# ilpoviertola/V-AURA

Measured on AMD Instinct MI355X. Metric: audio codec tokens/sec (whole node), 2.56 s clips, higher is better.
Workload: dtype f16x2-split(22b)/f32-acc

## Files before the change

### vaura_amd/csrc/dac.hip

```cpp
#include "common.h"
#include <algorithm>
#include <vector>

#define BM 128
#define BN 96
#define BK 32

struct ConvArgs {
  const float* in;
  const float* w;
  const float* bias;
  const float* res;
  const float* alpha;
  float* out_raw;
  float* out_act;
  int Lin, Lout, Cin, Cout, NT;
  int off_base, off_step;
  int ostride, oshift0;
  int jcount;
};

__host__ __device__ __forceinline__ size_t mx8_scale_offset(size_t elems) { return (elems + 15) & ~(size_t)15; }

#ifndef VA_CONV_ABL
// ... 128 lines not shown
  int off_base, off_step, ostride, oshift0, jcount;
  int act;
  int act_fmt;
  uint8_t* out_scale;
  const uint32_t* in_scale;
  const float* wscale;
  const uint16_t* w2;
  const float* bias2;
  const float* alpha_mid;
};

__device__ __forceinline__ float gelu_erf_f(float x) {
  if constexpr ((VA_CONV_ABL & 128) != 0) return 0.5f * x * (1.0f + x * 0.70710678118654752440f);
  if constexpr ((VA_CONV_ABL & 256) != 0) return 0.5f * x * (1.0f + erff(x * 0.70710678118654752440f));
  const float t = fabsf(x) * 0.70710678118654752440f;
  const float k = __builtin_amdgcn_rcpf(fmaf(t, 0.35f, 1.0f));
  float p = 0.06797561794519424f;
  p = fmaf(p, k, -0.4044332206249237f);
  p = fmaf(p, k, 0.8392713069915771f);
  p = fmaf(p, k, -0.7225478887557983f);
  p = fmaf(p, k, 0.6403822898864746f);
  p = fmaf(p, k, -0.046077974140644073f);
  p = fmaf(p, k, 0.23748238384723663f);
  p = fmaf(p, k, 0.1900186985731125f);
  p = fmaf(p, k, 0.1979287713766098f);
  const float e = (k * p) * __builtin_amdgcn_exp2f(-(t * t) * 1.4426950408889634f);
  return (0.5f * x) * (x < 0.f ? e : 2.0f - e);
}

__device__ __forceinline__ void store_pair4(uint16_t* base, size_t row, int c0, int C, const f32x4 v) {
  _Float16 h[4], l[4];
#pragma unroll
  for (int i = 0; i < 4; ++i) {
    const float x = v[i];
    h[i] = (_Float16)x;
    l[i] = (_Float16)(x - (float)h[i]);
  }
  typedef _Float16 f16x4 __attribute__((ext_vector_type(4)));
  f16x4* p = reinterpret_cast<f16x4*>(base + ((row * (size_t)(C >> 3) + (size_t)(c0 >> 3)) * 2) * 8 + (c0 & 7));
  p[0] = f16x4{h[0], h[1], h[2], h[3]};
  p[2] = f16x4{l[0], l[1], l[2], l[3]};
}

__device__ __forceinline__ int mx8_scale_byte(float amax) {
  const uint32_t bits = __builtin_bit_cast(uint32_t, amax);
  const int ea = (int)((bits >> 23) & 0xffu);
  const int e8 = ea - ((bits & 0x7fffffu) <= 0x600000u ? 8 : 7);
  return e8 < 1 ? 1 : (e8 > 253 ? 253 : e8);
}

__device__ __forceinline__ void store_act_octet(void* out_act, uint8_t* out_scale, int fmt, size_t grow, int co, int C,
                                                const float (&sv)[8]) {
  if (fmt == 0) {
    f16x8 hi, lo;
#pragma unroll
    for (int r = 0; r < 8; ++r) { hi[r] = (_Float16)sv[r]; lo[r] = (_Float16)(sv[r] - (float)hi[r]); }
    f16x8* dst = reinterpret_cast<f16x8*>(reinterpret_cast<uint16_t*>(out_act) + ((grow * (size_t)(C >> 3) + (size_t)(co >> 3)) * 2) * 8);
    dst[0] = hi;
    dst[1] = lo;
  } else {
    float amax = 0.f;
#pragma unroll
    for (int r = 0; r < 8; ++r) amax = fmaxf(amax, fabsf(sv[r]));
    amax = fmaxf(amax, __shfl_xor(amax, 1, 64));
    amax = fmaxf(amax, __shfl_xor(amax, 2, 64));
    const int e8 = mx8_scale_byte(amax);
    const float inv = __builtin_bit_cast(float, (uint32_t)(254 - e8) << 23);
    int q0 = 0, q1 = 0;
    q0 = __builtin_amdgcn_cvt_pk_fp8_f32(sv[0] * inv, sv[1] * inv, q0, false);
    q0 = __builtin_amdgcn_cvt_pk_fp8_f32(sv[2] * inv, sv[3] * inv, q0, true);
    q1 = __builtin_amdgcn_cvt_pk_fp8_f32(sv[4] * inv, sv[5] * inv, q1, false);
    q1 = __builtin_amdgcn_cvt_pk_fp8_f32(sv[6] * inv, sv[7] * inv, q1, true);
    typedef int i32x2 __attribute__((ext_vector_type(2)));
    *reinterpret_cast<i32x2*>(reinterpret_cast<uint8_t*>(out_act) + grow * (size_t)C + co) = i32x2{q0, q1};
    if (((co >> 3) & 3) == 0) out_scale[(grow * (size_t)((C + 127) >> 7) + (co >> 7)) * 4 + ((co >> 5) & 3)] = (uint8_t)e8;
  }
}

__device__ __forceinline__ float snake_fast(float v, float al) {
  const float sn = __builtin_amdgcn_sinf(__builtin_amdgcn_fractf(al * v * 0.15915494309189535f));
  return v + __builtin_amdgcn_rcpf(al + 1e-9f) * (sn * sn);
}

template <int BN_, int SP, bool FAST = false, int ROWS = BM>
__device__ __forceinline__ void conv_tile_store(const ConvPArgs& a, const float* stage, int b, int ph, int j0, int n0, int tid) {
  constexpr int OCT = BN_ / 8;
  static_assert(OCT % 4 == 0, "a 32-channel scale block = 4 consecutive threads of one row");
  constexpr int RSTEP = 256 / OCT;
  if (tid >= RSTEP * OCT) return;
  const int oc = tid % OCT, row0 = tid / OCT;
  const int co = n0 + oc * 8;
  const size_t obase = (size_t)b * a.Lout;
  f32x4 al0 = f32x4{0.f, 0.f, 0.f, 0.f}, al1 = al0, iv0 = al0, iv1 = al0;
  if (a.out_act && a.act == 0) {
    al0 = *reinterpret_cast<const f32x4*>(a.alpha + co);
    al1 = *reinterpret_cast<const f32x4*>(a.alpha + co + 4);
#pragma unroll
    for (int r = 0; r < 4; ++r) { iv0[r] = 1.0f / (al0[r] + 1e-9f); iv1[r] = 1.0f / (al1[r] + 1e-9f); }
  }
  for (int row = row0; row < ROWS; row += RSTEP) {
    const int jr = j0 + row;
    if (jr >= a.jcount) continue;
    const int orow = jr * a.ostride + a.oshift0 + ph;
    if (orow < 0 || orow >= a.Lout) continue;
    const size_t o = (obase + (size_t)orow) * a.Cout + co;
    f32x4 v0 = *reinterpret_cast<const f32x4*>(stage + row * SP + oc * 8);
    f32x4 v1 = *reinterpret_cast<const f32x4*>(stage + row * SP + oc * 8 + 4);
    if (a.res) {
      v0 = *reinterpret_cast<const f32x4*>(a.res + o) + v0;
      v1 = *reinterpret_cast<const f32x4*>(a.res + o + 4) + v1;
    }
    if (a.out_raw) {
      *reinterpret_cast<f32x4*>(a.out_raw + o) = v0;
      *reinterpret_cast<f32x4*>(a.out_raw + o + 4) = v1;
    }
    if (a.out_act) {
      float sv[8];
#pragma unroll
      for (int r = 0; r < 4; ++r) {
        if (FAST && a.act == 0) {
          sv[r] = snake_fast(v0[r], al0[r]);
          sv[r + 4] = snake_fast(v1[r], al1[r]);
        } else {
          sv[r] = a.act == 0 ? snake_fi(v0[r], al0[r], iv0[r]) : (a.act == 1 ? gelu_erf_f(v0[r]) : v0[r]);
          sv[r + 4] = a.act == 0 ? snake_fi(v1[r], al1[r], iv1[r]) : (a.act == 1 ? gelu_erf_f(v1[r]) : v1[r]);
        }
      }
      store_act_octet(a.out_act, a.out_scale, a.act_fmt, obase + (size_t)orow, co, a.Cout, sv);
    }
  }
}

#define XHALO 56
#define XROWS (BM + XHALO)
#ifndef VA_CONV_ABL
#define VA_CONV_ABL 0
#endif
template <int NI, bool WS, bool XS = false, int MJ = 4, bool FUSE = false>
__global__ __launch_bounds__(256, 2) void conv_pair_kernel(ConvPArgs a) {
  constexpr int BN_ = 32 * NI;
  constexpr int BMT = 32 * MJ;
  constexpr int XROWS_T = BMT + XHALO;
  constexpr int NXB = MJ == 4 ? 2 : 1;
  static_assert(MJ == 4 || MJ == 8, "128 or 256 rows");
  constexpr int WSTR = (BN_ + 3 + 15) / 16 * 16, XSTR = (XROWS_T + 3 + 15) / 16 * 16;
  constexpr int WS_ELEMS = 2 * (BK / 4) * WSTR, XS_ELEMS = NXB * (BK / 4) * XSTR;
  constexpr int SP = BN_ + 4;
  static_assert((WS_ELEMS + XS_ELEMS) * 16 >= BM * SP * 4, "the output tile must fit in the main loop's LDS");
  static_assert(!FUSE || (NI == 3 && MJ == 8), "the fused residual unit: all 96 channels in one 256-row workgroup");
  constexpr int W1STR = 112, YSTR = 80;
  constexpr int W1_ELEMS = FUSE ? 3 * (BK / 4) * W1STR : 0, Y_ELEMS = FUSE ? 3 * (BK / 4) * YSTR : 0;
  static_assert(!FUSE || Y_ELEMS * 16 >= 64 * SP * 4, "the 64-row output tile is staged over the activated tile");
  constexpr int SMEM_ELEMS = (WS_ELEMS + XS_ELEMS) > (W1_ELEMS + Y_ELEMS) ? (WS_ELEMS + XS_ELEMS) : (W1_ELEMS + Y_ELEMS);
  constexpr int TAB_ELEMS = FUSE ? 2 * BN_ / 4 : 0;
  __shared__ u32x4 smem[SMEM_ELEMS + TAB_ELEMS];
  auto coff = [](int kq) { return (kq & 1) + ((kq >> 2) << 1); };
  auto Ws = [&](int buf, int kq, int row) -> u32x4& { return smem[(buf * (BK / 4) + kq) * WSTR + row + coff(kq)]; };
  auto Xs = [&](int buf, int kq, int row) -> u32x4& { return smem[WS_ELEMS + (buf * (BK / 4) + kq) * XSTR + row + coff(kq)]; };
  const int tid = threadIdx.x, lane = tid & 63, wv = tid >> 6;
  const int wn = wv & 1, wm = wv >> 1;
  const int j0 = blockIdx.x * BMT;
  const int n0 = blockIdx.y * BN_;
  const int phases = a.ostride;
  const int b = blockIdx.z / phases, ph = blockIdx.z % phases;
  const int cq = a.Cin / 4;
  const u32x4* in = reinterpret_cast<const u32x4*>(a.in) + (size_t)b * a.Lin * cq;
  const u32x4* wbase = reinterpret_cast<const u32x4*>(a.w) + (size_t)ph * a.NT * a.Cout * cq;
  const int kc = a.Cin / BK;
  const int NT = a.NT;
  const int nk = NT * kc;
  const int span = (NT - 1) * (a.off_step < 0 ? -a.off_step : a.off_step);
  const int lo_off = a.off_base + (a.off_step < 0 ? (NT - 1) * a.off_step : 0);
  const int xrows = BMT + span;
  constexpr int XL = (XROWS_T * (BK / 4) + 255) / 256;

  u32x4 wreg[NI], xreg[XL];
  auto load_w = [&](int kt) {
    const int c = kt / NT, t = kt - c * NT;
    const u32x4* wt = wbase + (size_t)t * a.Cout * cq;
    const int q0 = c * (BK / 4);
#pragma unroll
    for (int i = 0; i < NI; ++i) {
      const int qd = tid + 256 * i, row = qd >> 3, kq = qd & 7;
      wreg[i] = wt[(size_t)(n0 + row) * cq + q0 + kq];
    }
  };
  auto store_w = [&](int buf) {
#pragma unroll
    for (int i = 0; i < NI; ++i) { const int qd = tid + 256 * i; Ws(buf, qd & 7, qd >> 3) = wreg[i]; }
  };
  auto load_x = [&](int c) {
    const int q0 = c * (BK / 4);
#pragma unroll
    for (int i = 0; i < XL; ++i) {
      const int qd = tid + 256 * i, row = qd >> 3, kq = qd & 7;
      const int jr = j0 + lo_off + row;
      xreg[i] = (row < xrows && jr >= 0 && jr < a.Lin) ? in[(size_t)jr * cq + q0 + kq] : u32x4{0u, 0u, 0u, 0u};
    }
  };
  auto store_x = [&](int buf) {
#pragma unroll
    for (int i = 0; i < XL; ++i) {
      const int qd = tid + 256 * i;
      if ((qd >> 3) < XROWS_T) Xs(buf, qd & 7, qd >> 3) = xreg[i];
    }
  };

  f32x4 acc[NI][MJ];
#pragma unroll
  for (int i = 0; i < NI; ++i)
#pragma unroll
    for (int j = 0; j < MJ; ++j) acc[i][j] = f32x4{0.f, 0.f, 0.f, 0.f};

  VA_STAMP_DECL(stamps);
  VA_STAMP(stamps, 0);
  load_w(0);
  load_x(0);
  store_w(0);
  store_x(0);
  if constexpr (FUSE) {
    if (tid < BN_) {
      float* tab = reinterpret_cast<float*>(smem + SMEM_ELEMS);
      const float al = a.alpha_mid[tid];
      tab[tid] = al;
      tab[BN_ + tid] = 1.0f / (al + 1e-9f);
    }
  }
  __syncthreads();
  VA_STAMP(stamps, 1);
  const int g = lane >> 4, r16 = lane & 15;
  int kt = 0;
  for (int c = 0; c < kc; ++c) {
    const int xb = NXB == 2 ? (c & 1) : 0;
    for (int t = 0; t < NT; ++t, ++kt) {
      const int buf = kt & 1;
      if (kt + 1 < nk && !(VA_CONV_ABL & 1)) load_w(kt + 1);
      if (t == (NXB == 2 ? 0 : NT - 1) && c + 1 < kc) load_x(c + 1);
      const int shift = (VA_CONV_ABL & 8) ? 0 : a.off_base + t * a.off_step - lo_off;
      f16x8 wh[NI], wl[NI];
#pragma unroll
      for (int i = 0; i < NI; ++i) {
        wh[i] = __builtin_bit_cast(f16x8, Ws(buf, 2 * g, wn * (NI * 16) + i * 16 + r16));
        if constexpr (!WS && !XS) wl[i] = __builtin_bit_cast(f16x8, Ws(buf, 2 * g + 1, wn * (NI * 16) + i * 16 + r16));
      }
      constexpr int JG = MJ == 4 ? 4 : 2;
#pragma unroll
      for (int jh = 0; jh < MJ; jh += JG) {
        f16x8 xh[JG], xl[JG];
#pragma unroll
        for (int j = 0; j < JG; ++j) {
          xh[j] = __builtin_bit_cast(f16x8, Xs(xb, 2 * g, shift + wm * (16 * MJ) + (jh + j) * 16 + r16));
          if constexpr (!XS) xl[j] = __builtin_bit_cast(f16x8, Xs(xb, 2 * g + 1, shift + wm * (16 * MJ) + (jh + j) * 16 + r16));
        }
#pragma unroll
        for (int i = 0; i < NI; ++i)
#pragma unroll
          for (int j = 0; j < JG; ++j) {
            if constexpr (VA_CONV_ABL & 2) {
              acc[i][jh + j][0] += (float)wh[i][0] * (float)xh[j][0];
              if constexpr (!XS) acc[i][jh + j][1] += (float)xl[j][0];
              if constexpr (!WS && !XS) acc[i][jh + j][2] += (float)wl[i][0];
              continue;
            }
            if constexpr (!WS && !XS) acc[i][jh + j] = __builtin_amdgcn_mfma_f32_16x16x32_f16(wl[i], xh[j], acc[i][jh + j], 0, 0, 0);
            if constexpr (!XS) acc[i][jh + j] = __builtin_amdgcn_mfma_f32_16x16x32_f16(wh[i], xl[j], acc[i][jh + j], 0, 0, 0);
            acc[i][jh + j] = __builtin_amdgcn_mfma_f32_16x16x32_f16(wh[i], xh[j], acc[i][jh + j], 0, 0, 0);
          }
      }
      if (kt + 1 < nk && !(VA_CONV_ABL & 1)) store_w(buf ^ 1);
      if (t == NT - 1 && c + 1 < kc) {
        if constexpr (NXB == 1) __syncthreads();
        store_x(NXB == 2 ? (xb ^ 1) : 0);
      }
      if constexpr (!(VA_CONV_ABL & 4)) __syncthreads();
    }
  }

  VA_STAMP(stamps, 2);
  if constexpr (FUSE) {
    u32x4* W1 = smem;
    u32x4* Yi = smem + W1_ELEMS;
    auto W1s = [&](int c2, int kq, int row) -> u32x4& { return W1[(c2 * (BK / 4) + kq) * W1STR + row + coff(kq)]; };
    auto Ys = [&](int c2, int kq, int row) -> u32x4& { return Yi[(c2 * (BK / 4) + kq) * YSTR + row + coff(kq)]; };
    u32x4 w1reg[9];
#pragma unroll
    for (int i = 0; i < 9; ++i) w1reg[i] = reinterpret_cast<const u32x4*>(a.w2)[tid + 256 * i];
    float* stage = reinterpret_cast<float*>(Yi);
    const float* tab = reinterpret_cast<const float*>(smem + SMEM_ELEMS);
    typedef _Float16 f16x4 __attribute__((ext_vector_type(4)));
    auto pass = [&](auto pc) {
      constexpr int p = decltype(pc)::value;
      if (p > 0) __syncthreads();
      if (wm == (p >> 1)) {
#pragma unroll
        for (int jj = 0; jj < 4; ++jj)
#pragma unroll
          for (int i = 0; i < NI; ++i) {
            const int col = wn * (NI * 16) + i * 16 + 4 * g;
            const f32x4 v = acc[i][4 * (p & 1) + jj] + *reinterpret_cast<const f32x4*>(a.bias + col);
            const f32x4 al = *reinterpret_cast<const f32x4*>(tab + col), iv = *reinterpret_cast<const f32x4*>(tab + BN_ + col);
            f16x4 h4, l4;
#pragma unroll
            for (int e = 0; e < 4; ++e) {
              const float sv = snake_fi(v[e], al[e], iv[e]);
              h4[e] = (_Float16)sv;
              l4[e] = (_Float16)(sv - (float)h4[e]);
            }
            const int c2 = col >> 5, o = (col & 31) >> 3, half = (col & 7) >> 2, row = jj * 16 + r16;
            reinterpret_cast<f16x4*>(&Ys(c2, 2 * o, row))[half] = h4;
            reinterpret_cast<f16x4*>(&Ys(c2, 2 * o + 1, row))[half] = l4;
          }
      }
      if (p == 0) {
#pragma unroll
        for (int i = 0; i < 9; ++i) {
          const int qd = tid + 256 * i, n = qd / 24, q = qd - n * 24;
          W1s(q >> 3, q & 7, n) = w1reg[i];
        }
      }
      __syncthreads();
      if (p == 0) VA_STAMP(stamps, 3);
      f32x4 acc2[NI][2];
#pragma unroll
      for (int i = 0; i < NI; ++i)
#pragma unroll
        for (int j = 0; j < 2; ++j) acc2[i][j] = f32x4{0.f, 0.f, 0.f, 0.f};
#pragma unroll
      for (int c2 = 0; c2 < 3; ++c2) {
        f16x8 wh[NI], wl[NI], xh[2], xl[2];
#pragma unroll
        for (int i = 0; i < NI; ++i) {
          wh[i] = __builtin_bit_cast(f16x8, W1s(c2, 2 * g, wn * (NI * 16) + i * 16 + r16));
          if constexpr (!WS && !XS) wl[i] = __builtin_bit_cast(f16x8, W1s(c2, 2 * g + 1, wn * (NI * 16) + i * 16 + r16));
        }
#pragma unroll
        for (int j = 0; j < 2; ++j) {
          xh[j] = __builtin_bit_cast(f16x8, Ys(c2, 2 * g, (wm * 2 + j) * 16 + r16));
          if constexpr (!XS) xl[j] = __builtin_bit_cast(f16x8, Ys(c2, 2 * g + 1, (wm * 2 + j) * 16 + r16));
        }
#pragma unroll
        for (int i = 0; i < NI; ++i)
#pragma unroll
          for (int j = 0; j < 2; ++j) {
            if constexpr (!WS && !XS) acc2[i][j] = __builtin_amdgcn_mfma_f32_16x16x32_f16(wl[i], xh[j], acc2[i][j], 0, 0, 0);
            if constexpr (!XS) acc2[i][j] = __builtin_amdgcn_mfma_f32_16x16x32_f16(wh[i], xl[j], acc2[i][j], 0, 0, 0);
            acc2[i][j] = __builtin_amdgcn_mfma_f32_16x16x32_f16(wh[i], xh[j], acc2[i][j], 0, 0, 0);
          }
      }
      __syncthreads();
      if (p == 0) VA_STAMP(stamps, 4);
#pragma unroll
      for (int i = 0; i < NI; ++i)
#pragma unroll
        for (int j = 0; j < 2; ++j) {
          const int row = (wm * 2 + j) * 16 + r16, col = wn * (NI * 16) + i * 16 + 4 * g;
          *reinterpret_cast<f32x4*>(stage + row * SP + col) = acc2[i][j] + *reinterpret_cast<const f32x4*>(a.bias2 + col);
        }
      __syncthreads();
      conv_tile_store<BN_, SP, false, 64>(a, stage, b, ph, j0 + p * 64, n0, tid);
      if (p == 0) VA_STAMP(stamps, 5);
    };
    pass(std::integral_constant<int, 0>{});
    pass(std::integral_constant<int, 1>{});
    pass(std::integral_constant<int, 2>{});
    pass(std::integral_constant<int, 3>{});
    VA_STAMP(stamps, 6);
    VA_STAMP_FLUSH(stamps, 21);
    return;
  }
  float* stage = reinterpret_cast<float*>(smem);
#pragma unroll
  for (int h = 0; h < MJ / 4; ++h) {
    if (h > 0) __syncthreads();
#pragma unroll
    for (int j = 0; j < MJ; ++j) {
      const int rbk = wm * MJ + j;
      if (rbk / 8 != h) continue;
#pragma unroll
      for (int i = 0; i < NI; ++i) {
        const int row = (rbk % 8) * 16 + r16, col = wn * (NI * 16) + i * 16 + 4 * g;
        *reinterpret_cast<f32x4*>(stage + row * SP + col) = acc[i][j] + *reinterpret_cast<const f32x4*>(a.bias + n0 + col);
      }
    }
    __syncthreads();
    if (h == 0) VA_STAMP(stamps, 4);
    conv_tile_store<BN_, SP>(a, stage, b, ph, j0 + h * BM, n0, tid);
    if (h == 0) VA_STAMP(stamps, 5);
  }
  VA_STAMP(stamps, 6);
  VA_STAMP_FLUSH(stamps, 20);
}

template <int N, typename F>
__device__ __forceinline__ void va_static_for(F&& f) {
  if constexpr (N > 0) {
    va_static_for<N - 1>(f);
    f(std::integral_constant<int, N - 1>{});
  }
}

template <int NCT, int RB, bool WS, bool XS>
__global__ __launch_bounds__(256, 2) void conv_unit_kernel(ConvPArgs a) {
  constexpr int C_ = 16 * NCT;
  constexpr int BMT = 64 * RB;
  constexpr int KC = C_ / BK;
  constexpr int XROWS_T = BMT + XHALO;
  constexpr int WSTR = (C_ + 3 + 15) / 16 * 16, XSTR = (XROWS_T + 3 + 15) / 16 * 16, W2STR = (BN + 3 + 15) / 16 * 16;
  constexpr int WS_ELEMS = 2 * (BK / 4) * WSTR, XS_ELEMS = (BK / 4) * XSTR;
  constexpr int SP = BN + 4;
  constexpr int W2_ELEMS = 2 * (BK / 4) * W2STR, ST_ELEMS = 64 * SP / 4;
  constexpr int MAIN_ELEMS = WS_ELEMS + XS_ELEMS > W2_ELEMS + ST_ELEMS ? WS_ELEMS + XS_ELEMS : W2_ELEMS + ST_ELEMS;
  constexpr int TAB_ELEMS = 2 * C_ / 4;
  static_assert(NCT % 6 == 0 && (RB == 2 || RB == 4) && NCT * RB == 24, "96 channels x 256 rows or 192 x 128: 96 accumulator registers");
  __shared__ u32x4 smem[MAIN_ELEMS + TAB_ELEMS];
  auto coff = [](int kq) { return (kq & 1) + ((kq >> 2) << 1); };
  auto Ws = [&](int buf, int kq, int row) -> u32x4& { return smem[(buf * (BK / 4) + kq) * WSTR + row + coff(kq)]; };
  auto Xs = [&](int kq, int row) -> u32x4& { return smem[WS_ELEMS + kq * XSTR + row + coff(kq)]; };
  auto W2s = [&](int buf, int kq, int row) -> u32x4& { return smem[(buf * (BK / 4) + kq) * W2STR + row + coff(kq)]; };
  float* tab = reinterpret_cast<float*>(smem + MAIN_ELEMS);
  const int tid = threadIdx.x, lane = tid & 63;
  const int wv = __builtin_amdgcn_readfirstlane(tid >> 6);
  const int g = lane >> 4, r16 = lane & 15;
  const int j0 = blockIdx.x * BMT, b = blockIdx.z;
  constexpr int cq = C_ / 4;
  const u32x4* in = reinterpret_cast<const u32x4*>(a.in) + (size_t)b * a.Lin * cq;
  const u32x4* wbase = reinterpret_cast<const u32x4*>(a.w);
  const int NT = a.NT, nk = NT * KC;
  const int span = (NT - 1) * (a.off_step < 0 ? -a.off_step : a.off_step);
  const int lo_off = a.off_base + (a.off_step < 0 ? (NT - 1) * a.off_step : 0);
  const int xrows = BMT + span;
  constexpr int WL = C_ * (BK / 4) / 256;
  constexpr int XL = (XROWS_T * (BK / 4) + 255) / 256;

  u32x4 wreg[WL], xreg[XL];
  auto load_w = [&](int kt) {
    const int c = kt / NT, t = kt - c * NT;
    const u32x4* wt = wbase + (size_t)t * C_ * cq + c * (BK / 4);
#pragma unroll
    for (int i = 0; i < WL; ++i) { const int qd = tid + 256 * i; wreg[i] = wt[(size_t)(qd >> 3) * cq + (qd & 7)]; }
  };
  auto store_w = [&](int buf) {
#pragma unroll
    for (int i = 0; i < WL; ++i) {
      const int qd = tid + 256 * i, ch = qd >> 3, w5 = ch & 31;
      Ws(buf, qd & 7, (ch & ~31) + (((w5 >> 2) & 1) << 4) + ((w5 >> 3) << 2) + (w5 & 3)) = wreg[i];
    }
  };
  auto load_x = [&](int c) {
#pragma unroll
    for (int i = 0; i < XL; ++i) {
      const int qd = tid + 256 * i, row = qd >> 3, kq = qd & 7;
      const int jr = j0 + lo_off + row;
      xreg[i] = (row < xrows && jr >= 0 && jr < a.Lin) ? in[(size_t)jr * cq + c * (BK / 4) + kq] : u32x4{0u, 0u, 0u, 0u};
    }
  };
  auto store_x = [&]() {
#pragma unroll
    for (int i = 0; i < XL; ++i) { const int qd = tid + 256 * i; if ((qd >> 3) < XROWS_T) Xs(qd & 7, qd >> 3) = xreg[i]; }
  };

  f32x4 acc[NCT][RB];
#pragma unroll
  for (int i = 0; i < NCT; ++i)
#pragma unroll
    for (int j = 0; j < RB; ++j) acc[i][j] = f32x4{0.f, 0.f, 0.f, 0.f};

  VA_STAMP_DECL(stamps);
  VA_STAMP(stamps, 0);
  load_w(0);
  load_x(0);
  store_w(0);
  store_x();
  for (int ch = tid; ch < C_; ch += 256) {
// ... 403 lines not shown
      const f16x8* pp = reinterpret_cast<const f16x8*>(reinterpret_cast<const _Float16*>(act) + (((size_t)b * L + r) * oct + oc) * 16);
      const f16x8 h = pp[0], lo = pp[1];
#pragma unroll
      for (int e = 0; e < 8; ++e) x[e] = (float)h[e] + (float)lo[e];
    } else {
      const f32x4* pp = reinterpret_cast<const f32x4*>(act + ((size_t)b * L + r) * C + 8 * oc);
      const f32x4 a0 = pp[0], a1 = pp[1];
      x[0] = a0[0]; x[1] = a0[1]; x[2] = a0[2]; x[3] = a0[3]; x[4] = a1[0]; x[5] = a1[1]; x[6] = a1[2]; x[7] = a1[3];
    }
    *reinterpret_cast<f32x4*>(rows + rr * SR + 8 * oc) = f32x4{x[0], x[1], x[2], x[3]};
    *reinterpret_cast<f32x4*>(rows + rr * SR + 8 * oc + 4) = f32x4{x[4], x[5], x[6], x[7]};
  }
  __syncthreads();
  const int half = __builtin_amdgcn_readfirstlane(tid >> 7), lo_ = tid & 127;
  const int c0 = half * (C >> 1), c1 = c0 + (C >> 1);
  f32x4 d4 = f32x4{0.f, 0.f, 0.f, 0.f};
#pragma unroll
  for (int t = 0; t < 7; ++t) {
    const f32x4* xr = reinterpret_cast<const f32x4*>(rows + (lo_ + t) * SR + c0);
    const f32x4* wr = reinterpret_cast<const f32x4*>(w + (size_t)t * C + c0);
#pragma unroll 4
    for (int c = 0; c < (c1 - c0) / 4; ++c) {
      const f32x4 x = xr[c], ww = wr[c];
      d4[0] = fmaf(x[0], ww[0], d4[0]); d4[1] = fmaf(x[1], ww[1], d4[1]); d4[2] = fmaf(x[2], ww[2], d4[2]); d4[3] = fmaf(x[3], ww[3], d4[3]);
    }
  }
  const float d = (d4[0] + d4[1]) + (d4[2] + d4[3]);
  float* part = rows + (CO_TL + 6) * SR;
  if (half) part[lo_] = d;
  __syncthreads();
  if (!half && l0 + lo_ < L) wav[(size_t)b * L + l0 + lo_] = tanhf((d + part[lo_]) + bias[0]);
}

__global__ __launch_bounds__(256) void act_convert_kernel(const float* __restrict__ in, void* out, uint8_t* out_scale, size_t rows,
                                                          int C, int fmt) {
  const size_t u = (size_t)blockIdx.x * 256 + threadIdx.x;
  const int oct = C >> 3;
  const size_t row = u / oct;
  if (row >= rows) return;
  const int co = (int)(u - row * oct) * 8;
  const f32x4 v0 = *reinterpret_cast<const f32x4*>(in + row * C + co), v1 = *reinterpret_cast<const f32x4*>(in + row * C + co + 4);
  const float sv[8] = {v0[0], v0[1], v0[2], v0[3], v1[0], v1[1], v1[2], v1[3]};
  store_act_octet(out, out_scale, fmt, row, co, C, sv);
}

static long long va_conv256_launches = 0;

static int launch_conv(const vaura_conv& cv, const float* in, const float* res, const float* alpha, float* out_raw,
                       float* out_act, int B, int Lin, int pairs, hipStream_t s) {
  if (!cv.w || !cv.bias || (cv.cin % BK)) return VAURA_ERR_SHAPE;
  if (out_act && !alpha) return VAURA_ERR_ARG;
  if (pairs) {
    if ((cv.cout % BN) && (cv.cout % 64)) return VAURA_ERR_SHAPE;
    ConvPArgs p;
    p.in = reinterpret_cast<const uint16_t*>(in); p.w = reinterpret_cast<const uint16_t*>(cv.w); p.bias = cv.bias; p.res = res;
    p.alpha = alpha; p.out_raw = out_raw; p.out_act = reinterpret_cast<uint16_t*>(out_act);
    p.Lin = Lin; p.Cin = cv.cin; p.Cout = cv.cout; p.act = 0;
    p.act_fmt = 0; p.out_scale = nullptr; p.in_scale = nullptr; p.wscale = nullptr;
    p.w2 = nullptr; p.bias2 = nullptr; p.alpha_mid = nullptr;
    int ph = 1;
    if (cv.stride > 1) {
      if (cv.stride % 2) return VAURA_ERR_SHAPE;
      p.NT = 2; p.off_base = 0; p.off_step = -1; p.ostride = cv.stride; p.oshift0 = -(cv.stride / 2);
      p.Lout = Lin * cv.stride; p.jcount = Lin + 1; ph = cv.stride;
    } else {
      p.NT = cv.taps; p.off_base = -((cv.taps - 1) / 2) * cv.dilation; p.off_step = cv.dilation;
      p.ostride = 1; p.oshift0 = 0; p.Lout = Lin; p.jcount = Lin;
      if ((cv.taps - 1) * cv.dilation > XHALO) return VAURA_ERR_SHAPE;
    }
    if (pairs == 3) {
      if (out_act) {
        p.act_fmt = 1;
        p.out_scale = reinterpret_cast<uint8_t*>(out_act) + mx8_scale_offset((size_t)B * p.Lout * cv.cout);
      }
      if (cv.wscale) {
        if (cv.cout % BN) return VAURA_ERR_SHAPE;
        p.wscale = cv.wscale;
        p.in_scale = reinterpret_cast<const uint32_t*>(reinterpret_cast<const uint8_t*>(in) + mx8_scale_offset((size_t)B * Lin * cv.cin));
        VA_LAUNCH((conv_mx8_kernel<3>), dim3((p.jcount + BM - 1) / BM, cv.cout / BN, B * ph), dim3(256), 0, s, p);
        return 0;
      }
      pairs = 2;
    }
    if (pairs == 4) {
      const int g256 = (p.jcount + 2 * BM - 1) / (2 * BM);
      if (cv.cout % BN == 0 && !(va_debug_flags_get() & 0x100000u) && (int64_t)g256 * (cv.cout / BN) * B * ph >= 384) {
        ++va_conv256_launches;
        VA_LAUNCH((conv_pair_kernel<3, true, true, 8>), dim3(g256, cv.cout / BN, B * ph), dim3(256), 0, s, p);
      } else if (cv.cout % BN == 0) VA_LAUNCH((conv_pair_kernel<3, true, true>), dim3((p.jcount + BM - 1) / BM, cv.cout / BN, B * ph), dim3(256), 0, s, p);
      else VA_LAUNCH((conv_pair_kernel<2, true, true>), dim3((p.jcount + BM - 1) / BM, cv.cout / 64, B * ph), dim3(256), 0, s, p);
      return 0;
    }
    if (cv.cout % BN == 0) {
      const int g256 = (p.jcount + 2 * BM - 1) / (2 * BM);
      const bool big = !(va_debug_flags_get() & 0x100000u) && (int64_t)g256 * (cv.cout / BN) * B * ph >= 384;
      if (big) {
        ++va_conv256_launches;
        if (pairs == 2) VA_LAUNCH((conv_pair_kernel<3, true, false, 8>), dim3(g256, cv.cout / BN, B * ph), dim3(256), 0, s, p);
        else VA_LAUNCH((conv_pair_kernel<3, false, false, 8>), dim3(g256, cv.cout / BN, B * ph), dim3(256), 0, s, p);
      } else if (pairs == 2) VA_LAUNCH((conv_pair_kernel<3, true>), dim3((p.jcount + BM - 1) / BM, cv.cout / BN, B * ph), dim3(256), 0, s, p);
      else VA_LAUNCH((conv_pair_kernel<3, false>), dim3((p.jcount + BM - 1) / BM, cv.cout / BN, B * ph), dim3(256), 0, s, p);
    } else {
      const int g256 = (p.jcount + 2 * BM - 1) / (2 * BM);
      const bool big = !(va_debug_flags_get() & 0x100000u) && (int64_t)g256 * (cv.cout / 64) * B * ph >= 384;
      if (big) {
        ++va_conv256_launches;
        if (pairs == 2) VA_LAUNCH((conv_pair_kernel<2, true, false, 8>), dim3(g256, cv.cout / 64, B * ph), dim3(256), 0, s, p);
        else VA_LAUNCH((conv_pair_kernel<2, false, false, 8>), dim3(g256, cv.cout / 64, B * ph), dim3(256), 0, s, p);
      } else if (pairs == 2) VA_LAUNCH((conv_pair_kernel<2, true>), dim3((p.jcount + BM - 1) / BM, cv.cout / 64, B * ph), dim3(256), 0, s, p);
      else VA_LAUNCH((conv_pair_kernel<2, false>), dim3((p.jcount + BM - 1) / BM, cv.cout / 64, B * ph), dim3(256), 0, s, p);
    }
    return 0;
  }
  if (cv.cout % BN) return VAURA_ERR_SHAPE;
  ConvArgs a;
  a.in = in; a.w = cv.w; a.bias = cv.bias; a.res = res; a.alpha = alpha; a.out_raw = out_raw; a.out_act = out_act;
  a.Lin = Lin; a.Cin = cv.cin; a.Cout = cv.cout;
  int phases = 1;
  if (cv.stride > 1) {
    if (cv.stride % 2) return VAURA_ERR_SHAPE;
    a.NT = 2; a.off_base = 0; a.off_step = -1; a.ostride = cv.stride; a.oshift0 = -(cv.stride / 2);
    a.Lout = Lin * cv.stride; a.jcount = Lin + 1; phases = cv.stride;
  } else {
    a.NT = cv.taps; a.off_base = -((cv.taps - 1) / 2) * cv.dilation; a.off_step = cv.dilation;
    a.ostride = 1; a.oshift0 = 0; a.Lout = Lin; a.jcount = Lin;
  }
  dim3 grid((a.jcount + BM - 1) / BM, cv.cout / BN, B * phases);
  VA_LAUNCH(conv_mfma_kernel, grid, dim3(256), 0, s, a);
  return 0;
}


#define VA_UNIT_NOT_ELIGIBLE (-0x7fffff00)
static long long va_conv_units_fused = 0;
static int launch_conv_unit(const vaura_conv& c7, const vaura_conv& c1, const float* in, const float* res, const float* alpha_mid,
                            const float* alpha_next, float* out_raw, float* out_act, int B, int L, int pairs, hipStream_t s) {
  if (pairs != 1 && pairs != 2 && pairs != 4) return VA_UNIT_NOT_ELIGIBLE;
  if (va_debug_flags_get() & (0x200000u | 0x100000u)) return VA_UNIT_NOT_ELIGIBLE;
  const int C = c7.cin;
  if ((C != BN && C != 2 * BN) || c7.cout != C || c1.cin != C || c1.cout != C || c7.stride != 1 || c1.stride != 1 || c1.taps != 1 || c7.taps < 1 ||
      (c7.taps - 1) * c7.dilation > XHALO || !c7.w || !c7.bias || !c1.w || !c1.bias || !alpha_mid || !alpha_next || !res || !out_act || (const float*)out_act == in)
    return VA_UNIT_NOT_ELIGIBLE;
  const int rows = C == BN ? 256 : 128;
  const int gx = (L + rows - 1) / rows;
  if ((int64_t)gx * B < 384) return VA_UNIT_NOT_ELIGIBLE;
  ConvPArgs p;
  p.in = reinterpret_cast<const uint16_t*>(in); p.w = reinterpret_cast<const uint16_t*>(c7.w); p.bias = c7.bias; p.res = res;
  p.alpha = alpha_next; p.out_raw = out_raw; p.out_act = reinterpret_cast<uint16_t*>(out_act);
  p.Lin = L; p.Lout = L; p.Cin = C; p.Cout = C; p.act = 0;
  p.act_fmt = 0; p.out_scale = nullptr; p.in_scale = nullptr; p.wscale = nullptr;
  p.NT = c7.taps; p.off_base = -((c7.taps - 1) / 2) * c7.dilation; p.off_step = c7.dilation;
  p.ostride = 1; p.oshift0 = 0; p.jcount = L;
  p.w2 = reinterpret_cast<const uint16_t*>(c1.w); p.bias2 = c1.bias; p.alpha_mid = alpha_mid;
  ++va_conv_units_fused;
  const dim3 grid(gx, 1, B);
  if (C == BN) {
    if (pairs == 4) VA_LAUNCH((conv_pair_kernel<3, true, true, 8, true>), grid, dim3(256), 0, s, p);
    else if (pairs == 2) VA_LAUNCH((conv_pair_kernel<3, true, false, 8, true>), grid, dim3(256), 0, s, p);
    else VA_LAUNCH((conv_pair_kernel<3, false, false, 8, true>), grid, dim3(256), 0, s, p);
  } else {
    if (pairs == 4) VA_LAUNCH((conv_unit_kernel<12, 2, true, true>), grid, dim3(256), 0, s, p);
    else if (pairs == 2) VA_LAUNCH((conv_unit_kernel<12, 2, true, false>), grid, dim3(256), 0, s, p);
    else VA_LAUNCH((conv_unit_kernel<12, 2, false, false>), grid, dim3(256), 0, s, p);
  }
  return 0;
}


#define LBN 192
#ifndef VA_LIN_ABL
#define VA_LIN_ABL 0
#endif
template <int MW>
__global__ __launch_bounds__(128 * MW, MW == 2 ? 2 : 1) void linear_pair_kernel(ConvPArgs a, int mtiles, int ntiles) {
  constexpr int NTH = 128 * MW, LBM_ = 64 * MW, NWQ = LBN * 8 / NTH, NXQ = LBM_ * 8 / NTH;
  __shared__ u32x4 smem[8 * (LBN + LBM_)];
  auto Ws = [&](int kq, int row) -> u32x4& { return smem[kq * LBN + (row ^ kq)]; };
  auto Xs = [&](int kq, int row) -> u32x4& { return smem[8 * LBN + kq * LBM_ + (row ^ kq)]; };
  const int tid = threadIdx.x, lane = tid & 63, wv = tid >> 6;
  const int wn = wv & 1, wm = wv >> 1;
  const int xcd = blockIdx.x & 7, local = blockIdx.x >> 3;
  const int nt = local % ntiles, mt = (local / ntiles) * 8 + xcd;
  if (mt >= mtiles) return;
  const int b = blockIdx.y;
  const int j0 = mt * LBM_, n0 = nt * LBN;
  const int cq = a.Cin / 4;
// ... 1122 lines not shown
```

Baseline: 74740.

## Add few-tap pipelined schedule and remapped grid for 256-row conv kernels

Factors the conv pair kernel into a shared body and adds an XO variant for convolutions with one or two taps (strided or pointwise). That variant uses a single X buffer, prefetches the next input chunk into registers, and places sched barriers around the MFMA work so loads overlap compute. For stride-1 layers it also reorders the grid so that eight consecutive x-blocks share z, which changes which workgroups run together. The fused residual epilogue now splits rows across both wm halves with 32-row interleaving, so all waves store in every pass. The new paths add code complexity and depend on batch-divisibility conditions for the grid remap.

Result: no change. 74790, median of 4 (+0.1%).

```diff
diff --git a/vaura_amd/csrc/dac.hip b/vaura_amd/csrc/dac.hip
--- a/vaura_amd/csrc/dac.hip
+++ b/vaura_amd/csrc/dac.hip
@@ -234,7 +234,7 @@
   return v + __builtin_amdgcn_rcpf(al + 1e-9f) * (sn * sn);
 }
 
-template <int BN_, int SP, bool FAST = false, int ROWS = BM>
+template <int BN_, int SP, bool FAST = false, int ROWS = BM, int SPLIT = 0>
 __device__ __forceinline__ void conv_tile_store(const ConvPArgs& a, const float* stage, int b, int ph, int j0, int n0, int tid) {
   constexpr int OCT = BN_ / 8;
   static_assert(OCT % 4 == 0, "a 32-channel scale block = 4 consecutive threads of one row");
@@ -251,7 +251,7 @@
     for (int r = 0; r < 4; ++r) { iv0[r] = 1.0f / (al0[r] + 1e-9f); iv1[r] = 1.0f / (al1[r] + 1e-9f); }
   }
   for (int row = row0; row < ROWS; row += RSTEP) {
-    const int jr = j0 + row;
+    const int jr = j0 + row + (SPLIT > 0 && row >= SPLIT ? BM - SPLIT : 0);
     if (jr >= a.jcount) continue;
     const int orow = jr * a.ostride + a.oshift0 + ph;
     if (orow < 0 || orow >= a.Lout) continue;
@@ -288,8 +288,9 @@
 #ifndef VA_CONV_ABL
 #define VA_CONV_ABL 0
 #endif
-template <int NI, bool WS, bool XS = false, int MJ = 4, bool FUSE = false>
-__global__ __launch_bounds__(256, 2) void conv_pair_kernel(ConvPArgs a) {
+template <int NI, bool WS, bool XS, int MJ, bool FUSE, bool XO>
+__device__ __forceinline__ void conv_pair_body(const ConvPArgs& a) {
+  static_assert(!XO || (MJ == 8 && !FUSE), "the few-tap schedule belongs to the 256-row conv instances");
   constexpr int BN_ = 32 * NI;
   constexpr int BMT = 32 * MJ;
   constexpr int XROWS_T = BMT + XHALO;
@@ -311,10 +312,18 @@
   auto Xs = [&](int buf, int kq, int row) -> u32x4& { return smem[WS_ELEMS + (buf * (BK / 4) + kq) * XSTR + row + coff(kq)]; };
   const int tid = threadIdx.x, lane = tid & 63, wv = tid >> 6;
   const int wn = wv & 1, wm = wv >> 1;
-  const int j0 = blockIdx.x * BMT;
+  int bx = blockIdx.x, bz = blockIdx.z;
+  if constexpr (XO) {
+    if (a.ostride == 1) {
+      const int gx = (a.jcount + BMT - 1) / BMT, rt = blockIdx.z * 8 + blockIdx.x;
+      bz = rt / gx;
+      bx = rt - bz * gx;
+    }
+  }
+  const int j0 = bx * BMT;
   const int n0 = blockIdx.y * BN_;
   const int phases = a.ostride;
-  const int b = blockIdx.z / phases, ph = blockIdx.z % phases;
+  const int b = bz / phases, ph = bz % phases;
   const int cq = a.Cin / 4;
   const u32x4* in = reinterpret_cast<const u32x4*>(a.in) + (size_t)b * a.Lin * cq;
   const u32x4* wbase = reinterpret_cast<const u32x4*>(a.w) + (size_t)ph * a.NT * a.Cout * cq;
@@ -381,50 +390,122 @@
   __syncthreads();
   VA_STAMP(stamps, 1);
   const int g = lane >> 4, r16 = lane & 15;
-  int kt = 0;
-  for (int c = 0; c < kc; ++c) {
-    const int xb = NXB == 2 ? (c & 1) : 0;
-    for (int t = 0; t < NT; ++t, ++kt) {
-      const int buf = kt & 1;
-      if (kt + 1 < nk && !(VA_CONV_ABL & 1)) load_w(kt + 1);
-      if (t == (NXB == 2 ? 0 : NT - 1) && c + 1 < kc) load_x(c + 1);
-      const int shift = (VA_CONV_ABL & 8) ? 0 : a.off_base + t * a.off_step - lo_off;
-      f16x8 wh[NI], wl[NI];
-#pragma unroll
-      for (int i = 0; i < NI; ++i) {
-        wh[i] = __builtin_bit_cast(f16x8, Ws(buf, 2 * g, wn * (NI * 16) + i * 16 + r16));
-        if constexpr (!WS && !XS) wl[i] = __builtin_bit_cast(f16x8, Ws(buf, 2 * g + 1, wn * (NI * 16) + i * 16 + r16));
-      }
-      constexpr int JG = MJ == 4 ? 4 : 2;
-#pragma unroll
-      for (int jh = 0; jh < MJ; jh += JG) {
-        f16x8 xh[JG], xl[JG];
+  auto mma = [&](int buf, int xb, int shift) {
+    f16x8 wh[NI], wl[NI];
+#pragma unroll
+    for (int i = 0; i < NI; ++i) {
+      wh[i] = __builtin_bit_cast(f16x8, Ws(buf, 2 * g, wn * (NI * 16) + i * 16 + r16));
+      if constexpr (!WS && !XS) wl[i] = __builtin_bit_cast(f16x8, Ws(buf, 2 * g + 1, wn * (NI * 16) + i * 16 + r16));
+    }
+    constexpr int JG = MJ == 4 ? 4 : 2;
+#pragma unroll
+    for (int jh = 0; jh < MJ; jh += JG) {
+      f16x8 xh[JG], xl[JG];
+#pragma unroll
+      for (int j = 0; j < JG; ++j) {
+        xh[j] = __builtin_bit_cast(f16x8, Xs(xb, 2 * g, shift + wm * (16 * MJ) + (jh + j) * 16 + r16));
+        if constexpr (!XS) xl[j] = __builtin_bit_cast(f16x8, Xs(xb, 2 * g + 1, shift + wm * (16 * MJ) + (jh + j) * 16 + r16));
+      }
+#pragma unroll
+      for (int i = 0; i < NI; ++i)
 #pragma unroll
         for (int j = 0; j < JG; ++j) {
-          xh[j] = __builtin_bit_cast(f16x8, Xs(xb, 2 * g, shift + wm * (16 * MJ) + (jh + j) * 16 + r16));
-          if constexpr (!XS) xl[j] = __builtin_bit_cast(f16x8, Xs(xb, 2 * g + 1, shift + wm * (16 * MJ) + (jh + j) * 16 + r16));
+          if constexpr (VA_CONV_ABL & 2) {
+            acc[i][jh + j][0] += (float)wh[i][0] * (float)xh[j][0];
+            if constexpr (!XS) acc[i][jh + j][1] += (float)xl[j][0];
+            if constexpr (!WS && !XS) acc[i][jh + j][2] += (float)wl[i][0];
+            continue;
+          }
+          if constexpr (!WS && !XS) acc[i][jh + j] = __builtin_amdgcn_mfma_f32_16x16x32_f16(wl[i], xh[j], acc[i][jh + j], 0, 0, 0);
+          if constexpr (!XS) acc[i][jh + j] = __builtin_amdgcn_mfma_f32_16x16x32_f16(wh[i], xl[j], acc[i][jh + j], 0, 0, 0);
+          acc[i][jh + j] = __builtin_amdgcn_mfma_f32_16x16x32_f16(wh[i], xh[j], acc[i][jh + j], 0, 0, 0);
         }
-#pragma unroll
-        for (int i = 0; i < NI; ++i)
-#pragma unroll
-          for (int j = 0; j < JG; ++j) {
-            if constexpr (VA_CONV_ABL & 2) {
-              acc[i][jh + j][0] += (float)wh[i][0] * (float)xh[j][0];
-              if constexpr (!XS) acc[i][jh + j][1] += (float)xl[j][0];
-              if constexpr (!WS && !XS) acc[i][jh + j][2] += (float)wl[i][0];
-              continue;
-            }
-            if constexpr (!WS && !XS) acc[i][jh + j] = __builtin_amdgcn_mfma_f32_16x16x32_f16(wl[i], xh[j], acc[i][jh + j], 0, 0, 0);
-            if constexpr (!XS) acc[i][jh + j] = __builtin_amdgcn_mfma_f32_16x16x32_f16(wh[i], xl[j], acc[i][jh + j], 0, 0, 0);
-            acc[i][jh + j] = __builtin_amdgcn_mfma_f32_16x16x32_f16(wh[i], xh[j], acc[i][jh + j], 0, 0, 0);
+    }
+  };
+  if constexpr (XO) {
+    auto few = [&](auto ntc) {
+      constexpr int NTC = decltype(ntc)::value;
+      constexpr int NQ = (BMT + NTC - 1) * (BK / 4) / 256 + (NTC > 1 ? 1 : 0);
+      u32x4 xr[NQ];
+      auto ldx = [&](int c) {
+        const u32x4* src = in + c * (BK / 4);
+        int z = 0;
+        asm volatile("" : "+s"(z));
+#pragma unroll
+        for (int i = 0; i < NQ; ++i) {
+          const int qd = tid + 256 * i, row = qd >> 3, kq = qd & 7;
+          int jr = j0 + lo_off + z + (row < xrows ? row : xrows - 1);
+          jr = jr < 0 ? 0 : (jr >= a.Lin ? a.Lin - 1 : jr);
+          xr[i] = src[(unsigned)(jr * cq + kq)];
+        }
+      };
+      auto stx = [&]() {
+#pragma unroll
+        for (int i = 0; i < NQ; ++i) {
+          const int qd = tid + 256 * i, row = qd >> 3, jr = j0 + lo_off + row;
+          if (i < BMT / 32 || row < xrows) Xs(0, qd & 7, row) = (jr >= 0 && jr < a.Lin) ? xr[i] : u32x4{0u, 0u, 0u, 0u};
+        }
+      };
+      const int sh0 = a.off_base - lo_off, sh1 = a.off_base + a.off_step - lo_off;
+      auto chunk = [&](int c, auto more_c) {
+        constexpr bool more = decltype(more_c)::value;
+        if constexpr (NTC == 1) {
+          if constexpr (more) {
+            load_w(c + 1);
+            ldx(c + 1);
+            __builtin_amdgcn_sched_barrier(0);
           }
-      }
-      if (kt + 1 < nk && !(VA_CONV_ABL & 1)) store_w(buf ^ 1);
-      if (t == NT - 1 && c + 1 < kc) {
-        if constexpr (NXB == 1) __syncthreads();
-        store_x(NXB == 2 ? (xb ^ 1) : 0);
-      }
-      if constexpr (!(VA_CONV_ABL & 4)) __syncthreads();
+          mma(c & 1, 0, sh0);
+          __builtin_amdgcn_sched_barrier(0);
+          if constexpr (more) {
+            store_w((c & 1) ^ 1);
+            __syncthreads();
+            stx();
+          }
+          __syncthreads();
+        } else {
+          load_w(2 * c + 1);
+          if constexpr (more) ldx(c + 1);
+          __builtin_amdgcn_sched_barrier(0);
+          mma(0, 0, sh0);
+          store_w(1);
+          __syncthreads();
+          if constexpr (more) {
+            load_w(2 * c + 2);
+            __builtin_amdgcn_sched_barrier(0);
+          }
+          mma(1, 0, sh1);
+          __builtin_amdgcn_sched_barrier(0);
+          if constexpr (more) {
+            store_w(0);
+            __syncthreads();
+            stx();
+          }
+          __syncthreads();
+        }
+      };
+      for (int c = 0; c + 1 < kc; ++c) chunk(c, std::true_type{});
+      chunk(kc - 1, std::false_type{});
+    };
+    if (NT == 1) few(std::integral_constant<int, 1>{});
+    else few(std::integral_constant<int, 2>{});
+  } else {
+    int kt = 0;
+    for (int c = 0; c < kc; ++c) {
+      const int xb = NXB == 2 ? (c & 1) : 0;
+      for (int t = 0; t < NT; ++t, ++kt) {
+        const int buf = kt & 1;
+        if (kt + 1 < nk && !(VA_CONV_ABL & 1)) load_w(kt + 1);
+        if (t == (NXB == 2 ? 0 : NT - 1) && c + 1 < kc) load_x(c + 1);
+        const int shift = (VA_CONV_ABL & 8) ? 0 : a.off_base + t * a.off_step - lo_off;
+        mma(buf, xb, shift);
+        if (kt + 1 < nk && !(VA_CONV_ABL & 1)) store_w(buf ^ 1);
+        if (t == NT - 1 && c + 1 < kc) {
+          if constexpr (NXB == 1) __syncthreads();
+          store_x(NXB == 2 ? (xb ^ 1) : 0);
+        }
+        if constexpr (!(VA_CONV_ABL & 4)) __syncthreads();
+      }
     }
   }
 
@@ -443,13 +524,13 @@
     auto pass = [&](auto pc) {
       constexpr int p = decltype(pc)::value;
       if (p > 0) __syncthreads();
-      if (wm == (p >> 1)) {
-#pragma unroll
-        for (int jj = 0; jj < 4; ++jj)
+      {
+#pragma unroll
+        for (int jj = 0; jj < 2; ++jj)
 #pragma unroll
           for (int i = 0; i < NI; ++i) {
             const int col = wn * (NI * 16) + i * 16 + 4 * g;
-            const f32x4 v = acc[i][4 * (p & 1) + jj] + *reinterpret_cast<const f32x4*>(a.bias + col);
+            const f32x4 v = acc[i][2 * p + jj] + *reinterpret_cast<const f32x4*>(a.bias + col);
             const f32x4 al = *reinterpret_cast<const f32x4*>(tab + col), iv = *reinterpret_cast<const f32x4*>(tab + BN_ + col);
             f16x4 h4, l4;
 #pragma unroll
@@ -458,7 +539,7 @@
               h4[e] = (_Float16)sv;
               l4[e] = (_Float16)(sv - (float)h4[e]);
             }
-            const int c2 = col >> 5, o = (col & 31) >> 3, half = (col & 7) >> 2, row = jj * 16 + r16;
+            const int c2 = col >> 5, o = (col & 31) >> 3, half = (col & 7) >> 2, row = wm * 32 + jj * 16 + r16;
             reinterpret_cast<f16x4*>(&Ys(c2, 2 * o, row))[half] = h4;
             reinterpret_cast<f16x4*>(&Ys(c2, 2 * o + 1, row))[half] = l4;
           }
@@ -509,7 +590,7 @@
           *reinterpret_cast<f32x4*>(stage + row * SP + col) = acc2[i][j] + *reinterpret_cast<const f32x4*>(a.bias2 + col);
         }
       __syncthreads();
-      conv_tile_store<BN_, SP, false, 64>(a, stage, b, ph, j0 + p * 64, n0, tid);
+      conv_tile_store<BN_, SP, false, 64, 32>(a, stage, b, ph, j0 + p * 32, n0, tid);
       if (p == 0) VA_STAMP(stamps, 5);
     };
     pass(std::integral_constant<int, 0>{});
@@ -541,6 +622,15 @@
   }
   VA_STAMP(stamps, 6);
   VA_STAMP_FLUSH(stamps, 20);
+}
+
+template <int NI, bool WS, bool XS = false, int MJ = 4, bool FUSE = false>
+__global__ __launch_bounds__(256, 2) void conv_pair_kernel(ConvPArgs a) {
+  conv_pair_body<NI, WS, XS, MJ, FUSE, false>(a);
+}
+template <bool WS, bool XS>
+__global__ __launch_bounds__(256, 2) void conv_pair_xo_kernel(ConvPArgs a) {
+  conv_pair_body<3, WS, XS, 8, false, true>(a);
 }
 
 template <int N, typename F>
@@ -1110,26 +1200,30 @@
       }
       pairs = 2;
     }
+    const int g256 = (p.jcount + 2 * BM - 1) / (2 * BM);
+    const bool few = cv.stride > 1 || cv.taps == 1;
+    const bool xo = !(va_debug_flags_get() & 0x1000u) && few && (ph > 1 || ((int64_t)g256 * B) % 8 == 0);
+    const dim3 grid256 = xo && ph == 1 ? dim3(8, cv.cout / BN, (unsigned)((int64_t)g256 * B / 8)) : dim3(g256, cv.cout / BN, B * ph);
     if (pairs == 4) {
-      const int g256 = (p.jcount + 2 * BM - 1) / (2 * BM);
       if (cv.cout % BN == 0 && !(va_debug_flags_get() & 0x100000u) && (int64_t)g256 * (cv.cout / BN) * B * ph >= 384) {
         ++va_conv256_launches;
-        VA_LAUNCH((conv_pair_kernel<3, true, true, 8>), dim3(g256, cv.cout / BN, B * ph), dim3(256), 0, s, p);
+        if (xo) VA_LAUNCH((conv_pair_xo_kernel<true, true>), grid256, dim3(256), 0, s, p);
+        else VA_LAUNCH((conv_pair_kernel<3, true, true, 8>), grid256, dim3(256), 0, s, p);
       } else if (cv.cout % BN == 0) VA_LAUNCH((conv_pair_kernel<3, true, true>), dim3((p.jcount + BM - 1) / BM, cv.cout / BN, B * ph), dim3(256), 0, s, p);
       else VA_LAUNCH((conv_pair_kernel<2, true, true>), dim3((p.jcount + BM - 1) / BM, cv.cout / 64, B * ph), dim3(256), 0, s, p);
       return 0;
     }
     if (cv.cout % BN == 0) {
-      const int g256 = (p.jcount + 2 * BM - 1) / (2 * BM);
       const bool big = !(va_debug_flags_get() & 0x100000u) && (int64_t)g256 * (cv.cout / BN) * B * ph >= 384;
       if (big) {
         ++va_conv256_launches;
-        if (pairs == 2) VA_LAUNCH((conv_pair_kernel<3, true, false, 8>), dim3(g256, cv.cout / BN, B * ph), dim3(256), 0, s, p);
-        else VA_LAUNCH((conv_pair_kernel<3, false, false, 8>), dim3(g256, cv.cout / BN, B * ph), dim3(256), 0, s, p);
+        if (pairs == 2 && xo) VA_LAUNCH((conv_pair_xo_kernel<true, false>), grid256, dim3(256), 0, s, p);
+        else if (pairs == 2) VA_LAUNCH((conv_pair_kernel<3, true, false, 8>), grid256, dim3(256), 0, s, p);
+        else if (xo) VA_LAUNCH((conv_pair_xo_kernel<false, false>), grid256, dim3(256), 0, s, p);
+        else VA_LAUNCH((conv_pair_kernel<3, false, false, 8>), grid256, dim3(256), 0, s, p);
       } else if (pairs == 2) VA_LAUNCH((conv_pair_kernel<3, true>), dim3((p.jcount + BM - 1) / BM, cv.cout / BN, B * ph), dim3(256), 0, s, p);
       else VA_LAUNCH((conv_pair_kernel<3, false>), dim3((p.jcount + BM - 1) / BM, cv.cout / BN, B * ph), dim3(256), 0, s, p);
     } else {
-      const int g256 = (p.jcount + 2 * BM - 1) / (2 * BM);
       const bool big = !(va_debug_flags_get() & 0x100000u) && (int64_t)g256 * (cv.cout / 64) * B * ph >= 384;
       if (big) {
         ++va_conv256_launches;
```
